# cvxgrp/qcqp

Measured on AMD Instinct MI355X. Metric: restarts x coord-sweeps / sec (improve COORD_DESCENT phase-2 sweeps, 2n^2 flops each; whole step timed), higher is better.
Workload: dtype f64

## Files before the change

qcqp_amd/csrc/cd_life.hip:

```cpp
#include "cd_life.h"

#include <cstdio>
#include <cstdlib>

#include "onevar.h"
#include "cd_phase1_sep.h"
#include "cd_chain.h"
#include "cd_roles.h"

namespace qcqpmi {
namespace {

constexpr int L2_WD = 1 << 21;
enum { L2_ABORT = 3 };

__device__ __attribute__((always_inline)) inline RqOwn l2_own(int NB, int CS, int m, int NMW) {
    RqOwn o;
    const int rest = NB - CS;
    o.NB = NB;
    if (m < 0) { o.first = rest; o.stride = 1; o.nu = CS; }
    else { o.first = m; o.stride = NMW; o.nu = m < rest ? (rest - m + NMW - 1) / NMW : 0; }
    return o;
}

constexpr int L2_SHARED_DOUBLES = 8 + 8 + 16 + 8;
constexpr int L2_YU = 6;
constexpr int l2_tile_doubles(int nmw, int csu, int lr, int kcl = 1, int maxc = 1) {
    return 2 * nmw * 256 + 256 + 256 + 2 * 256 + 2 * 48 + 4 * 256 + csu * 256 + 16 + 8 + 16 * 4 + 8 * 5 + 64 * 10 + 16 * 3 + 8 * 5 + 32 +
           (lr ? L2_YBMAX * 256 + 2 * 256 : 0) +
           2 * (maxc + 1) * 16 * kcl + 2 * 8 * kcl + (kcl > 1 ? 16 : 0);
}
#define L2_LDS_VIEW(tile_) \
    extern __shared__ double smem[]; \
    int *ctl = (int *)smem; \
    int *simdof = (int *)(smem + 8); \
    int *p1cols = (int *)(smem + 16); \
    int *jn = (int *)(smem + 32); \
    double *sp = smem + L2_SHARED_DOUBLES + (tile_) * l2_tile_doubles(NMW, CSU, LRV, KCLV, MAXC); \
    double *part2 = sp; sp += 2 * NMW * 256; \
    double *fixp = sp; sp += 256; \
    double *gtile = sp; sp += 256; \
    double *DU2 = sp; sp += 2 * 256; \
    double *sc2 = sp; sp += 2 * 48; \
    double *ring = sp; sp += 4 * 256; \
    double *cshare = sp; sp += CSU * 256; \
    double *slk = sp; sp += 16; \
    rq_lds_int *sy = (rq_lds_int *)(int *)sp; sp += 8; \
    double *of0 = sp; sp += 16; \
    long long *ovis = (long long *)sp; sp += 16; \
    long long *oacc = (long long *)sp; sp += 16; \
    long long *oswp = (long long *)sp; sp += 16; \
    int *sid = (int *)sp; sp += 8; \
    int *snew = (int *)sp; sp += 8; \
    int *sfin = (int *)sp; sp += 8; \
    int *ost = (int *)sp; sp += 8; \
    int *gatep = (int *)sp; sp += 8; \
    long long *cst = (long long *)sp; sp += 64 * 10; \
    unsigned long long *sseed = (unsigned long long *)sp; sp += 16; \
    unsigned long long *sfirst = (unsigned long long *)sp; sp += 16; \
    unsigned long long *p1key = (unsigned long long *)sp; sp += 16; \
    int *p1upd = (int *)sp; sp += 8; \
    int *p1fin = (int *)sp; sp += 8; \
    int *p1sw = (int *)sp; sp += 8; \
    int *p1st = (int *)sp; sp += 8; \
    L2Par *par = (L2Par *)sp; sp += 32;       \
    double *ytile = sp; sp += LRV ? L2_YBMAX * 256 : 0; \
    double *pend = sp; sp += LRV ? 2 * 256 : 0; \
    SetTable<MAXC> TC;        \
    TC.slots = 16 * KCLV; \
    TC.lo = sp; sp += (MAXC + 1) * 16 * KCLV; \
    TC.hi = sp; sp += (MAXC + 1) * 16 * KCLV; \
    TC.n = (int *)sp; sp += 8 * KCLV; \
    TC.slow = (int *)sp; sp += 8 * KCLV; \
    int *clsb = (int *)sp;
template <class T>
__device__ __attribute__((always_inline)) inline T *l2_tl(T *p, int t, int tile_doubles) { return (T *)((double *)p + t * tile_doubles); }

struct L2Par {
    const double *Apack, *Apack2, *Dpack, *Spack;
    const double *Gpack, *Upack;
    int RB, pad_;
    double *Xg;
    int *next;
    unsigned long long *prof;
    long long num_iters, n16;
    double tol, r0, fbound;
    int NB, KS, n, nlast, Rtotal, dbg;
    const int *cls;
};
static_assert(sizeof(L2Par) <= 32 * sizeof(double), "L2Par outgrew its LDS slot");
__device__ __attribute__((always_inline)) inline int l2_uni(int v) { return __builtin_amdgcn_readfirstlane(v); }
__device__ __attribute__((always_inline)) inline long long l2_uni(long long v) {
    const int lo = __builtin_amdgcn_readfirstlane((int)(v & 0xffffffffll)), hi = __builtin_amdgcn_readfirstlane((int)(v >> 32));
    return ((long long)hi << 32) | (long long)(unsigned)lo;
}
__device__ __attribute__((always_inline)) inline double l2_uni(double v) { return __longlong_as_double(l2_uni(__double_as_longlong(v))); }
template <class T>
__device__ __attribute__((always_inline)) inline T *l2_uni(T *p) { return (T *)(uintptr_t)l2_uni((long long)(uintptr_t)p); }

template <int NMW, int CS>
__device__ __attribute__((noinline)) void l2_mfma_role(int m_in, int t_in) {
    constexpr int MAXC = 1;
    constexpr int KCLV = 1;
    constexpr int CSU = CS > 0 ? CS : 1;
    constexpr int LRV = 0;
    const int tile = l2_uni(t_in);
    L2_LDS_VIEW(tile)
    (void)ytile; (void)pend; (void)clsb;
    (void)fixp; (void)gtile; (void)DU2; (void)sc2; (void)cshare; (void)slk; (void)TC; (void)of0; (void)ovis; (void)oacc; (void)oswp; (void)sid; (void)snew;
    (void)sfin; (void)ost; (void)ctl; (void)cst; (void)sseed; (void)sfirst; (void)p1key; (void)p1upd; (void)p1fin; (void)p1sw; (void)p1st; (void)gatep; (void)simdof; (void)p1cols; (void)jn;
    const int lane = threadIdx.x & 63;
    const int m = l2_uni(m_in);
    const double *pApack2 = l2_uni(par->Apack2);
    double *pXg = l2_uni(par->Xg);
    unsigned long long *pprof = l2_uni(par->prof);
    const int NB = l2_uni(par->NB), KS = l2_uni(par->KS);
    const int64_t n16 = l2_uni(par->n16);
    const int rowmask = (l2_uni(par->dbg) & 1) ? 7 : -1;
    const int64_t gmax = (int64_t)1 << 40;
    const RqOwn own = l2_own(NB, CS, m, NMW);
    const int nu = own.nu;
    v2d_ arP[2 * RQ_PFU];
    const unsigned vlane = (unsigned)lane * 16u;
    const __amdgpu_buffer_rsrc_t arsrc = __builtin_amdgcn_make_buffer_rsrc(const_cast<double *>(pApack2), 0, NB * KS * 512, 0x00020000);
    const __amdgpu_buffer_rsrc_t xrsrc = __builtin_amdgcn_make_buffer_rsrc(pXg, 0, (int)(n16 * 128), 0x00020000);
    const int rowstride = KS * 512;
    typedef unsigned rq_u4 __attribute__((ext_vector_type(4)));
    typedef unsigned rq_u2 __attribute__((ext_vector_type(2)));
    #define L2_LDA(dst, soff, vo) { const rq_u4 t0_ = __builtin_amdgcn_raw_buffer_load_b128(arsrc, (vo), (soff), 0);           \
                            const rq_u4 t1_ = __builtin_amdgcn_raw_buffer_load_b128(arsrc, (vo) + 1024u, (soff), 0);   \
                            (dst)[0] = __builtin_bit_cast(v2d_, t0_); (dst)[1] = __builtin_bit_cast(v2d_, t1_); }
    double bq[4 * RQ_PERS];
    {
        const unsigned vl8 = (unsigned)lane * 8u;
    #pragma unroll
        for (int u = 0; u < RQ_PERS; u++)
    #pragma unroll
            for (int q = 0; q < 4; q++) {
                const rq_u2 t_ = __builtin_amdgcn_raw_buffer_load_b64(xrsrc, vl8, (m + NMW * u) * 2048 + q * 512, 0);
                bq[4 * u + q] = __builtin_bit_cast(double, t_);
            }
    }
    typedef __attribute__((address_space(3))) const double rq_lds_cd;
    rq_lds_cd *rbase = (rq_lds_cd *)(ring + lane);
    asm volatile("" : "+v"(rbase));
    int row = 0;
    #pragma unroll
    for (int U = 0; U < RQ_PFU; U++) L2_LDA(arP + 2 * U, row * rowstride + (m + ((U < nu) ? NMW * U : 0)) * 2048, vlane)
    int spins = 0;
    const bool prof_on = pprof != nullptr && m == 0 && tile == 0;
    long long pw_commit = 0, pw_cons = 0;
    for (int64_t i = 0; i < gmax; i++) {
        const int row2 = (row + 1 == NB) ? 0 : row + 1;
        const int h1 = row == 0 ? NB - 1 : row - 1;
        const int h2 = h1 == 0 ? NB - 1 : h1 - 1;
        const int r1 = (i >= 3) ? (h2 == 0 ? NB - 1 : h2 - 1) : -1;
        unsigned skip = ~0u << own.nu, fresh = 0u;
        if (h1 % NMW == m && h1 < NB - CS) skip |= 1u << (h1 / NMW);
        if (h2 % NMW == m && h2 < NB - CS) skip |= 1u << (h2 / NMW);
        if (r1 >= 0 && r1 % NMW == m && r1 < NB - CS) fresh |= 1u << (r1 / NMW);
        const int so1 = (row & rowmask) * rowstride + m * 2048, so2 = (row2 & rowmask) * rowstride + m * 2048;
        bool stop = false;
        if (i >= 3) {
            const long long tw0 = prof_on ? (long long)__builtin_amdgcn_s_memtime() : 0;
            for (;;) {
                const rq_i4 s4 = rq_sync_read(sy);
                if (s4[RQ_STOP]) { stop = true; break; }
                if (s4[RQ_COMMIT] >= (int)i - 2) break;
                if (++spins > L2_WD) { stop = true; rq_sync_write(sy, L2_ABORT, 1, lane); rq_sync_write(sy, RQ_STOP, 1, lane); break; }
                __builtin_amdgcn_s_sleep(1);
            }
            if (stop) break;
            spins = 0;
            if (prof_on) pw_commit += (long long)__builtin_amdgcn_s_memtime() - tw0;
            if (fresh) {
                rq_lds_cd *rp = rbase + (int)((i - 3) & 3) * 256;
    #pragma unroll
                for (int u = 0; u < RQ_PERS; u++)
                    if ((fresh >> u) & 1u) {
    #pragma unroll
                        for (int q = 0; q < 4; q++) bq[4 * u + q] = rp[q * 64];
                    }
            }
        }
        v4d_ acc = {0.0, 0.0, 0.0, 0.0}, acc1 = acc;
    #pragma unroll
        for (int third = 0; third < RQ_RND; third++) {
    #pragma unroll
            for (int U = 0; U < RQ_PFU; U++) {
                const int u = RQ_PFU * third + U;
                if (u < RQ_MAXU && !((skip >> u) & 1u)) {
                    const double *bu = bq + 4 * u;
                    acc = __builtin_amdgcn_mfma_f64_16x16x4f64(arP[2 * U][0], bu[0], acc, 0, 0, 0);
                    acc1 = __builtin_amdgcn_mfma_f64_16x16x4f64(arP[2 * U][1], bu[1], acc1, 0, 0, 0);
                    acc = __builtin_amdgcn_mfma_f64_16x16x4f64(arP[2 * U + 1][0], bu[2], acc, 0, 0, 0);
                    acc1 = __builtin_amdgcn_mfma_f64_16x16x4f64(arP[2 * U + 1][1], bu[3], acc1, 0, 0, 0);
                }
                if (third < RQ_RND - 1) { if (u + RQ_PFU < RQ_MAXU) L2_LDA(arP + 2 * U, so1 + ((u + RQ_PFU < nu) ? NMW * 2048 * (u + RQ_PFU) : 0), vlane) }
                else L2_LDA(arP + 2 * U, so2 + ((U < nu) ? NMW * 2048 * U : 0), vlane)
            }
        }
        acc = acc + acc1;
        if (i >= 2) {
            const long long tw0 = prof_on ? (long long)__builtin_amdgcn_s_memtime() : 0;
            for (;;) {
                const rq_i4 s4 = rq_sync_read(sy);
                if (s4[RQ_STOP]) { stop = true; break; }
                if (s4[RQ_CONS] >= (int)i - 1) break;
                if (++spins > L2_WD) { stop = true; rq_sync_write(sy, L2_ABORT, 1, lane); rq_sync_write(sy, RQ_STOP, 1, lane); break; }
                __builtin_amdgcn_s_sleep(1);
            }
            if (stop) break;
            spins = 0;
            if (prof_on) pw_cons += (long long)__builtin_amdgcn_s_memtime() - tw0;
        }
        {
            double *part = part2 + (int)(i & 1) * NMW * 256 + m * 256;
    #pragma unroll
            for (int v = 0; v < 4; v++) part[v * 64 + (lane & 15) * 4 + (lane >> 4)] = acc[v];
        }
        rq_sync_write(sy, RQ_PARTS + m, (int)i + 1, lane);
        row = row2;
    }
    if (prof_on && lane == 0) {
        atomicAdd(pprof + 9, (unsigned long long)pw_commit);
        atomicAdd(pprof + 10, (unsigned long long)pw_cons);
    }
    #undef L2_LDA
}


template <int NMW>
__device__ __attribute__((noinline)) void l2_mfma_lr_role(int m_in, int t_in) {
    constexpr int MAXC = 1;
    constexpr int KCLV = 1;
    constexpr int CSU = 1;
    constexpr int LRV = 1;
    constexpr int YU = L2_YU;
    const int tile = l2_uni(t_in);
    L2_LDS_VIEW(tile)
    (void)clsb;
    (void)fixp; (void)gtile; (void)DU2; (void)sc2; (void)cshare; (void)slk; (void)TC; (void)of0; (void)ovis; (void)oacc; (void)oswp; (void)sid; (void)snew;
    (void)sfin; (void)ost; (void)ctl; (void)cst; (void)sseed; (void)sfirst; (void)p1key; (void)p1upd; (void)p1fin; (void)p1sw; (void)p1st; (void)gatep; (void)simdof; (void)p1cols; (void)jn;
// ... 560 lines not shown
                }
                double bqC[4 * CSU];
    #pragma unroll
                for (int U = 0; U < CSU; U++)
    #pragma unroll
                    for (int q = 0; q < 4; q++) bqC[4 * U + q] = cshare[U * 256 + q * 64 + lane];
                acc = rq_product<CSU>(arC, bqC, Apk2, KS, cown, lane, us, rq_slot(cown, bprev), bn2, acc);
            }
    #pragma unroll
            for (int v = 0; v < 4; v++) fixp[v * 64 + (lane & 15) * 4 + (lane >> 4)] = acc[v];
        }
        {
            const int nx = (int)((g + 1) & 1);
    #pragma unroll
            for (int e = 0; e < 4; e++) DU2[nx * 256 + lane + 64 * e] = d4[e];
            if (lane < 48) sc2[nx * 48 + lane] = s3;
            if (MULTI && lane < 16) clsb[nx * 16 + lane] = c3;
        }
        L2_TICK(pt_fix)
        b = bn;
    }
#undef L2_TICK
    if (LR) {
        const int g1 = (int)((last_g - 1) & 3), g0 = (int)(last_g & 3);
        double p1v[4], p0v[4];
#pragma unroll
        for (int u = 0; u < 4; u++) { p1v[u] = ring[g1 * 256 + u * 64 + lane]; p0v[u] = ring[g0 * 256 + u * 64 + lane]; }
#pragma unroll
        for (int u = 0; u < 4; u++) { pend[u * 64 + lane] = p1v[u]; pend[256 + u * 64 + lane] = p0v[u]; }
    }
    rq_sync_write(sy, RQ_STOP, 1, lane);
    if (prof_on && lane == 0) {
        atomicAdd(pprof + 13, (unsigned long long)pt_sum);
        atomicAdd(pprof + 14, (unsigned long long)pt_steps);
        atomicAdd(pprof + 15, (unsigned long long)pt_end);
        atomicAdd(pprof + 19, (unsigned long long)pt_req);
        *(long long *)(ctl + 8) = (long long)__builtin_amdgcn_s_memtime();
        atomicAdd(pprof + 7, (unsigned long long)pt_fix);
        atomicAdd(pprof + 8, (unsigned long long)pw_part);
        atomicAdd(pprof + 11, (unsigned long long)pn_int);
        atomicAdd(pprof + 12, (unsigned long long)pn_gen);
    }
    {
        cst[0 * 64 + lane] = S.upd_counter; cst[1 * 64 + lane] = S.visits; cst[2 * 64 + lane] = S.accepted;
        cst[3 * 64 + lane] = S.sweeps; cst[4 * 64 + lane] = S.conv ? 1 : 0; cst[5 * 64 + lane] = S.status;
        cst[6 * 64 + lane] = __double_as_longlong(fpart);
        cst[7 * 64 + lane] = (frz ? 1 : 0) | (done ? 2 : 0) | (pre ? 4 : 0) | (ld ? 8 : 0);
        cst[8 * 64 + lane] = __double_as_longlong(facc);
        const double ftot = rq_quad_sum(facc) + P.r0;
        const bool fin = occupied && done;
        if (gq == 0) {
            sfin[r] = fin ? 1 : 0;
            if (fin) { ovis[r] = S.visits; oacc[r] = S.accepted; oswp[r] = S.sweeps; ost[r] = S.status; of0[r] = ftot; }
        }
    }
    __builtin_amdgcn_s_setprio(0);
}

template <int NMW, int CS, int KIND, int TILES, int LR>
__global__ __launch_bounds__((NMW == 3 && TILES == 1) ? 256 : 512, 2) void cd_life_kernel(CdLife2Args a0) {
    const CdLife2Args &a = a0;
    constexpr bool MULTI = KIND == L2_KIND_GENK || KIND == L2_KIND_LINK;
    constexpr int BK = KIND == L2_KIND_GENK ? L2_KIND_GEN : KIND == L2_KIND_LINK ? L2_KIND_LIN : KIND;
    constexpr int MAXC = MULTI ? 2 : 1;
    constexpr int KCLV = MULTI ? L2_KCL : 1;
    constexpr int CSU = CS > 0 ? CS : 1;
    constexpr int LRV = LR;
    static_assert(!MULTI || (TILES == 1 && !LR), "multi-class kinds: one tile per workgroup, no objective factor");
    constexpr int NT = (NMW == 3 && TILES == 1) ? 256 : 512;
    constexpr int NW = NT / 64;
    constexpr int NS = 16 * TILES;
    constexpr int TD = l2_tile_doubles(NMW, CSU, LR);
    static_assert(!LR || (NMW == 3 && CS == 0 && BK != L2_KIND_LIN && BK != L2_KIND_SGN), "factored objective: three multiplying waves per tile, no chain share, a positive diagonal");
    constexpr bool PRE = BK == L2_KIND_LIN || BK == L2_KIND_SGN;
    static_assert(TILES == 1 || NMW == 3, "two tiles per workgroup: eight waves = two chains + two x three multiplying waves");
    const DevProblem &P = a.P;
    const int tid0 = threadIdx.x;
    const int wave = __builtin_amdgcn_readfirstlane(tid0 >> 6);
    const int64_t n16 = P.n16;
    const int NB = (int)P.NB, KS = (int)P.KS;
    L2_LDS_VIEW(0)
    (void)fixp; (void)gtile; (void)DU2; (void)sc2; (void)ring; (void)cshare; (void)of0; (void)ovis; (void)oacc; (void)oswp; (void)ost; (void)ytile; (void)pend; (void)clsb;
#define L2_STORE_SETS(st_, sc_, slack_) {                                                                                              \
        SetTable<MAXC> T2 = TC;                                                                                                          \
        T2.lo = l2_tl(TC.lo, st_, TD); T2.hi = l2_tl(TC.hi, st_, TD); T2.n = l2_tl(TC.n, st_, TD); T2.slow = l2_tl(TC.slow, st_, TD);    \
        const int nk_ = MULTI ? a0.nclass : 1;                                                                                           \
        for (int k_ = 0; k_ < nk_; k_++) {                                                                                               \
            FeasSet<MAXC> C_;                                                                                                            \
            compute_set<MAXC>(P, P.krep[k_], slack_, C_);                                                                                \
            store_set<MAXC>(T2, 16 * k_ + (sc_), C_);                                                                                    \
            if (MULTI && C_.n > 2) T2.slow[16 * k_ + (sc_)] = 1;                                                                         \
        }                                                                                                                                \
    }
    GLB double *Xg0 = glb(a0.scratch) + (int64_t)blockIdx.x * TILES * n16 * 16;

    if ((tid0 & 63) == 0) simdof[wave] = (int)(__builtin_amdgcn_s_getreg(4 | (4 << 6) | (1 << 11)));
    if (NMW == 3 && TILES == 1 && tid0 == 0) {
        int arrival = 0;
        if (a0.cuslot) {
            const unsigned hw = __builtin_amdgcn_s_getreg(4 | (0 << 6) | (31 << 11)), xcc = __builtin_amdgcn_s_getreg(20 | (0 << 6) | (31 << 11));
            arrival = glb_add(glb(a0.cuslot) + (((xcc & 15) << 8) | (((hw >> 12) & 15) << 4) | ((hw >> 8) & 15)), 1);
        }
        simdof[8] = (arrival & 1) ? (a0.rotmode == 2 ? 16 + 1 : 2) : 0;
    }
    if (tid0 < 64 * TILES) {
        long long *cs_ = l2_tl(cst, tid0 >> 6, TD);
#pragma unroll
        for (int f = 0; f < 10; f++) cs_[f * 64 + (tid0 & 63)] = (f == 4) ? 1 : 0;
    }
    if (tid0 < NS) { l2_tl(sid, tid0 >> 4, TD)[tid0 & 15] = -1; l2_tl(sfin, tid0 >> 4, TD)[tid0 & 15] = 0; }
    GLB const CdLife *lf0 = glb(a0.life);
    const long long life_t0 = (tid0 == 0 && lf0->prof) ? (long long)__builtin_amdgcn_s_memtime() : 0;
    __syncthreads();
    int role, rtile = 0;
    {
        int cnt[4] = {0, 0, 0, 0};
        int rank = 0;
        const int mys = simdof[wave];
#pragma unroll
        for (int w = 0; w < NW; w++) {
            const int s = simdof[w];
#pragma unroll
            for (int q = 0; q < 4; q++) cnt[q] += (s == q) ? 1 : 0;
            rank += (s == mys && w < wave) ? 1 : 0;
        }
        const bool even = cnt[0] == NW / 4 && cnt[1] == NW / 4 && cnt[2] == NW / 4 && cnt[3] == NW / 4;
        if (NMW == 3 && TILES == 1) {
            const int rot = simdof[8];
            if (!even) role = wave;
            else if (rot >= 16) role = mys == 0 ? 0 : 1 + ((mys - 1 + (rot - 16)) % 3);
            else role = (mys + rot) & 3;
        }
        else if (TILES == 2) { role = even ? mys : (wave & 3); rtile = even ? rank : (wave >> 2); }
        else if (even) role = (mys == 0) ? (rank == 0 ? 0 : 7) : mys + 3 * rank;
        else role = wave;
        role = __builtin_amdgcn_readfirstlane(role);
        rtile = __builtin_amdgcn_readfirstlane(rtile);
        if (tid0 == 0 && lf0->prof) {
            if (even) atomicAdd((unsigned long long *)lf0->prof + 6, 1ull);
            const unsigned hw = __builtin_amdgcn_s_getreg(4 | (0 << 6) | (31 << 11)), xcc = __builtin_amdgcn_s_getreg(20 | (0 << 6) | (31 << 11));
            Xg0[0] = (double)(((xcc & 15) << 8) | (((hw >> 13) & 7) << 4) | ((hw >> 8) & 15));
        }
    }
    const int nlast = (int)(P.n - 16 * (int64_t)(NB - 1));
    if (tid0 < TILES) {
        L2Par *pr = l2_tl(par, tid0, TD);
        pr->Apack = P.Apack; pr->Apack2 = P.Apack2; pr->Dpack = a0.Dpack; pr->Spack = a0.Spack;
        pr->Gpack = a0.Gpack; pr->Upack = a0.Upack; pr->RB = a0.RB; pr->pad_ = 0;
        pr->Xg = a0.scratch + ((int64_t)blockIdx.x * TILES + tid0) * n16 * 16; pr->next = a0.b.next; pr->prof = (unsigned long long *)lf0->prof;
        pr->num_iters = a.num_iters; pr->n16 = n16; pr->tol = a.tol; pr->r0 = P.r0; pr->fbound = a.fbound;
        pr->NB = NB; pr->KS = KS; pr->n = (int)P.n; pr->nlast = nlast; pr->Rtotal = (int)lf0->Rtotal; pr->dbg = a0.dbg;
        pr->cls = P.cls;
    }
    __syncthreads();

    for (;;) {
        int tid = tid0;
        asm volatile("" : "+v"(tid));
        const CdLife *lifep = a0.life;
        asm volatile("" : "+s"(lifep));
        const int lane = tid & 63, r = lane >> 2;
        if (tid == 0) { ctl[0] = 0; jn[0] = 0; jn[1] = 0; }
        __syncthreads();
        if (tid < NS) {
            const int st = tid >> 4, sc = tid & 15;
            int id = l2_tl(sid, st, TD)[sc], nw = 0;
            if (id < 0) {
                GLB const CdLife *lf = glb(lifep);
                const int idx = glb_add(glb(a0.b.next), 1);
                if (idx < (int)lf->Rtotal) {
                    id = idx; nw = 1;
                    const uint64_t pop = (uint64_t)idx / (uint64_t)lf->Rpop, rho = (uint64_t)idx % (uint64_t)lf->Rpop;
                    l2_tl(sseed, st, TD)[sc] = lf->seed + pop * lf->seed_stride;
                    l2_tl(sfirst, st, TD)[sc] = lf->first_index + pop * lf->first_stride + rho - (uint64_t)idx;
                }
            }
            l2_tl(sid, st, TD)[sc] = id; l2_tl(snew, st, TD)[sc] = nw;
            if (nw) { l2_tl(p1fin, st, TD)[sc] = 0; l2_tl(p1sw, st, TD)[sc] = 0; l2_tl(p1st, st, TD)[sc] = 0; l2_tl(gatep, st, TD)[sc] = 0; }
            if (id < 0) {
                l2_tl(slk, st, TD)[sc] = 0.0;
                L2_STORE_SETS(st, sc, 0.0)
            }
            if (id >= 0) atomicAdd(&ctl[0], 1);
            *(volatile rq_lds_int *)(l2_tl((int *)sy, st, TD) + sc) = (sc >= RQ_PARTS + NMW) ? 0x7fffffff : 0;
        }
        __syncthreads();
        if (ctl[0] == 0) break;
        {
            __builtin_amdgcn_s_setprio(3);
            GLB const CdLife *lf = glb(lifep);
            const long long pt0 = lf->prof ? (long long)__builtin_amdgcn_s_memtime() : 0;
            const int lf_pre = LR ? lf->prebuilt : 0;
            const int lf_generate = lf->generate && !lf_pre, lf_phase1 = lf->phase1 && !lf_pre;
            const double lf_viol_tol = lf->viol_tol;
            const int e0 = P.cptr[P.krep[0]];
            const double cp = P.cp[e0], cq = P.cq[e0], cr = P.cr[e0];
            const int rel = P.crel[e0];
            for (int c = 0; c < NS; c++) {
                const int ct = c >> 4, cc = c & 15;
                GLB double *Xg = Xg0 + (int64_t)ct * n16 * 16;
                if (!l2_tl(snew, ct, TD)[cc]) {
                    if (l2_tl(sid, ct, TD)[cc] < 0) for (int64_t j = tid; j < n16; j += NT) Xg[j * 16 + cc] = 0.0;
                    continue;
                }
                if (!lf_generate) {
                    const int id = l2_tl(sid, ct, TD)[cc];
                    GLB const double *src = glb(a0.b.X) + ((int64_t)(id >> 4) * n16) * 16 + (id & 15);
                    for (int64_t j0 = tid; j0 < n16; j0 += 4 * NT) {
                        double t4[4];
#pragma unroll
                        for (int u = 0; u < 4; u++) t4[u] = (j0 + u * NT < n16) ? src[(j0 + u * NT) * 16] : 0.0;
#pragma unroll
                        for (int u = 0; u < 4; u++) if (j0 + u * NT < n16) Xg[(j0 + u * NT) * 16 + cc] = t4[u];
                    }
                }
            }
            if (lf_generate) {
                if (tid == 0) {
                    int cnt = 0;
                    for (int k = 0; k < NS; k++) if (l2_tl(snew, k >> 4, TD)[k & 15]) p1cols[cnt++] = k;
                    ctl[4] = cnt; ctl[5] = 0;
                }
                __syncthreads();
                const int ncolg = ctl[4], nchg = (int)((n16 + 127) / 128);
                for (;;) {
                    int ch = 0;
                    if (lane == 0) ch = atomicAdd(&ctl[5], 1);
                    ch = __builtin_amdgcn_readfirstlane(ch);
                    if (ch >= ncolg * nchg) break;
                    const int c = p1cols[ch / nchg], ct = c >> 4, cc = c & 15;
                    GLB double *Xg = Xg0 + (int64_t)ct * n16 * 16;
                    const int64_t j = (int64_t)(ch % nchg) * 128 + 2 * lane;
                    const uint64_t sd = l2_tl(sseed, ct, TD)[cc], gidx = l2_tl(sfirst, ct, TD)[cc] + (uint64_t)l2_tl(sid, ct, TD)[cc];
                    if (j < n16) {
                        double xo = 0.0;
                        const double xe = (j < P.n) ? keyed_normal_pair(sd, gidx, (uint64_t)j, &xo) : 0.0;
                        Xg[j * 16 + cc] = xe;
                        Xg[(j + 1) * 16 + cc] = (j + 1 < P.n) ? xo : 0.0;
                    }
                }
            }
            __syncthreads();
            if (lf->prof && tid == 0) atomicAdd((unsigned long long *)lf->prof + 4, (unsigned long long)((long long)__builtin_amdgcn_s_memtime() - pt0));
            if (lf_phase1) {
                const bool band2 = !MULTI && cq == 0.0 && rel == RELOP_EQ && cp > 1e-4 && cr < -1e-3;
                const int cw = band2 ? 128 : 64;
                const int nch = (int)((P.n + cw - 1) / cw);
                for (int64_t t = 0; t < a.num_iters; t++) {
                    if (tid == 0) {
                        int cnt = 0;
                        for (int k = 0; k < NS; k++) if (l2_tl(snew, k >> 4, TD)[k & 15] && !l2_tl(p1fin, k >> 4, TD)[k & 15]) p1cols[cnt++] = k;
                        ctl[4] = cnt; ctl[5] = 0;
                    }
                    if (tid < NS) { l2_tl(p1key, tid >> 4, TD)[tid & 15] = ordered_key(-QM_INF); l2_tl(p1upd, tid >> 4, TD)[tid & 15] = 0; }
                    __syncthreads();
                    const int ncol1 = ctl[4];
                    if (ncol1 == 0) break;
                    for (;;) {
                        int ch = 0;
                        if (lane == 0) ch = atomicAdd(&ctl[5], 1);
                        ch = __builtin_amdgcn_readfirstlane(ch);
                        if (ch >= ncol1 * nch) break;
                        const int c = p1cols[ch / nch], ct = c >> 4, cc = c & 15;
                        GLB double *Xg = Xg0 + (int64_t)ct * n16 * 16;
                        const uint64_t sd = l2_tl(sseed, ct, TD)[cc], gidx = l2_tl(sfirst, ct, TD)[cc] + (uint64_t)l2_tl(sid, ct, TD)[cc];
                        double va = -QM_INF;
                        int fl = 0;
                        if (band2) {
                            const int64_t i2[2] = {(int64_t)(ch % nch) * 128 + lane, (int64_t)(ch % nch) * 128 + 64 + lane};
                            const bool on2[2] = {i2[0] < P.n, i2[1] < P.n};
                            double x2[2] = {on2[0] ? Xg[i2[0] * 16 + cc] : 1.0, on2[1] ? Xg[i2[1] * 16 + cc] : 1.0};
                            P1Visit V2[2];
                            p1_band_visit_n<2>(cp, cq, cr, i2, x2, on2, a.tol, lf_viol_tol, sd, gidx, t, V2);
#pragma unroll
                            for (int k = 0; k < 2; k++)
                                if (on2[k]) {
                                    if (V2[k].moved) { Xg[i2[k] * 16 + cc] = x2[k]; fl |= 1; }
                                    if (V2[k].status) fl |= (-V2[k].status) << 8;
                                    va = V2[k].vafter > va ? V2[k].vafter : va;
                                }
                        } else {
                            const int64_t i = (int64_t)(ch % nch) * 64 + lane;
                            if (i < P.n) {
                                if (MULTI) {
                                    double xi = Xg[i * 16 + cc];
                                    P1Visit V;
                                    p1_sep_visit<MAXC>(P, i, xi, a.tol, lf_viol_tol, sd, gidx, t, V);
                                    fl = (V.moved ? 1 : 0) | ((-V.status) << 8);
                                    va = V.vafter;
                                    if (V.moved) Xg[i * 16 + cc] = xi;
                                } else {
                                    const double xi = p1_class_visit(cp, cq, cr, rel, i, Xg[i * 16 + cc], a.tol, lf_viol_tol, sd, gidx, t, &fl, &va);
                                    if (fl & 1) Xg[i * 16 + cc] = xi;
                                }
                            }
                        }
                        const double vmax = wave_max(va);
                        const bool anyupd = __builtin_amdgcn_ballot_w64((fl & 1) != 0) != 0ull;
                        const int st = (fl >> 8) ? -(fl >> 8) : 0;
                        if (lane == 0) { atomicMax(&l2_tl(p1key, ct, TD)[cc], ordered_key(vmax)); if (anyupd) l2_tl(p1upd, ct, TD)[cc] = 1; }
                        if (st) l2_tl(p1st, ct, TD)[cc] = st;
                    }
                    __syncthreads();
                    if (tid < NS && l2_tl(snew, tid >> 4, TD)[tid & 15] && !l2_tl(p1fin, tid >> 4, TD)[tid & 15]) {
                        const int st = tid >> 4, sc = tid & 15;
                        l2_tl(p1sw, st, TD)[sc]++;
                        if (ordered_unkey(l2_tl(p1key, st, TD)[sc]) < lf_viol_tol || !l2_tl(p1upd, st, TD)[sc]) l2_tl(p1fin, st, TD)[sc] = 1;
                    }
                    __syncthreads();
                }
            }
            if (lf->prof && tid == 0) atomicAdd((unsigned long long *)lf->prof + 17, (unsigned long long)((long long)__builtin_amdgcn_s_memtime() - pt0));
            if (tid < NS) l2_tl(p1key, tid >> 4, TD)[tid & 15] = ordered_key(-QM_INF);
            __syncthreads();
            for (int c = 0; c < NS; c++) {
                const int ct = c >> 4, cc = c & 15;
                if (lf_pre || !l2_tl(snew, ct, TD)[cc]) continue;
                GLB const double *Xg = Xg0 + (int64_t)ct * n16 * 16;
                double v = -QM_INF;
                for (int64_t i = tid; i < P.n; i += NT) {
                    const double x = Xg[i * 16 + cc];
                    if (MULTI) {
                        for (int e = P.cptr[i]; e < P.cptr[i + 1]; e++) {
                            const double f = (P.cp[e] * x + P.cq[e]) * x + P.cr[e];
                            const double w = viol_of(f, P.crel[e]);
                            v = w > v ? w : v;
                        }
                    } else {
                        const double f = (cp * x + cq) * x + cr;
                        const double w = (rel == RELOP_EQ) ? fabs(f) : (f > 0.0 ? f : 0.0);
                        v = w > v ? w : v;
                    }
                }
                v = wave_max(v);
                if (lane == 0) atomicMax(&l2_tl(p1key, ct, TD)[cc], ordered_key(v));
            }
            __syncthreads();
            if (tid < NS && l2_tl(snew, tid >> 4, TD)[tid & 15]) {
                const int st = tid >> 4, sc = tid & 15;
                double mvx;
                if (lf_pre) {
                    const int id = l2_tl(sid, st, TD)[sc];
                    mvx = glb(lf->preslack)[id];
                    l2_tl(p1sw, st, TD)[sc] = (int)glb(lf->sweeps1)[id];
                    l2_tl(p1st, st, TD)[sc] = glb(lf->status1)[id];
                    l2_tl(gatep, st, TD)[sc] = glb(lf->ran2)[id];
                } else {
                    mvx = ordered_unkey(l2_tl(p1key, st, TD)[sc]);
                    l2_tl(gatep, st, TD)[sc] = (mvx < lf_viol_tol && l2_tl(p1st, st, TD)[sc] == 0) ? 1 : 0;
                }
                l2_tl(slk, st, TD)[sc] = mvx;
                L2_STORE_SETS(st, sc, mvx)
            }
            __syncthreads();
            if (nlast < 16) {
                for (int w = tid; w < NS * (16 - nlast); w += NT) {
                    const int c = w % NS, ct = c >> 4, cc = c & 15, row = w / NS;
                    if (l2_tl(snew, ct, TD)[cc] || l2_tl(sid, ct, TD)[cc] < 0) {
                        const int nn = l2_tl(TC.n, ct, TD)[cc];
                        double xp = 0.0;
                        if (BK == L2_KIND_BAND) xp = nn >= 2 ? l2_tl(TC.lo, ct, TD)[16 * KCLV + cc] : 0.0;
                        else if (BK == L2_KIND_GEN) xp = nn >= 1 ? l2_tl(TC.hi, ct, TD)[cc] : 0.0;
                        else xp = nn >= 2 ? l2_tl(TC.hi, ct, TD)[16 * KCLV + cc] : l2_tl(TC.hi, ct, TD)[cc];
                        if (!(xp == xp) || __builtin_isinf(xp)) xp = 0.0;
                        (Xg0 + (int64_t)ct * n16 * 16)[(P.n + row) * 16 + cc] = xp;
                    }
                }
                __syncthreads();
            }
            if (LR) {
                const int r16 = 16 * a0.RB;
                const int y0n = lf_pre ? (int)lf->y0_count : 0;
                GLB const double *y0g = glb(lf->y0);
                for (int w = tid; w < NS * (32 + r16); w += NT) {
                    const int c = w % NS, ct = c >> 4, cc = c & 15, rowz = w / NS;
                    const int id = l2_tl(sid, ct, TD)[cc];
                    if (l2_tl(snew, ct, TD)[cc] || id < 0) {
                        double v = 0.0;
                        if (id >= 0 && id < y0n)
                            v = rowz < 32 ? (Xg0 + (int64_t)ct * n16 * 16)[(16 * (int64_t)(NB - 2) + rowz) * 16 + cc]
                                          : y0g[((int64_t)(id >> 4) * r16 + (rowz - 32)) * 16 + (id & 15)];
                        if (rowz < 32) l2_tl(pend, ct, TD)[rowz * 16 + cc] = v;
                        else l2_tl(ytile, ct, TD)[(rowz - 32) * 16 + cc] = v;
                    }
                }
                __syncthreads();
            }
            if (lf->prof && tid == 0) {
                int nn = 0;
                for (int k = 0; k < NS; k++) nn += l2_tl(snew, k >> 4, TD)[k & 15] ? 1 : 0;
                atomicAdd((unsigned long long *)lf->prof + 0, (unsigned long long)((long long)__builtin_amdgcn_s_memtime() - pt0));
                atomicAdd((unsigned long long *)lf->prof + 2, 1ull);
                atomicAdd((unsigned long long *)lf->prof + 3, (unsigned long long)nn);
            }
            __builtin_amdgcn_s_setprio(0);
        }
        if (role == 0) {
            long long *cs_ = l2_tl(cst, rtile, TD);
            if (l2_tl(snew, rtile, TD)[r]) {
#pragma unroll
                for (int f = 0; f < 6; f++) cs_[f * 64 + lane] = 0;
                const int pass = l2_tl(gatep, rtile, TD)[r];
                bool load = LR != 0;
                if (LR) {
                    GLB const CdLife *lf = glb(lifep);
                    if (lf->prebuilt && l2_tl(sid, rtile, TD)[r] < (int)lf->y0_count) load = false;
                }
                cs_[6 * 64 + lane] = 0;
                cs_[4 * 64 + lane] = (pass && !PRE && !load) ? 0 : 1;
                cs_[7 * 64 + lane] = (pass ? (PRE ? 4 : 0) : 1) | (load ? 8 : 0);
                cs_[8 * 64 + lane] = 0;
            } else if (l2_tl(sid, rtile, TD)[r] < 0) {
                cs_[4 * 64 + lane] = 1; cs_[6 * 64 + lane] = 0;
                cs_[7 * 64 + lane] = 2; cs_[8 * 64 + lane] = 0;
            }
        }
        __syncthreads();
        if (tid == 0 && glb(lifep)->prof) *(long long *)(ctl + 6) = (long long)__builtin_amdgcn_s_memtime();

        if (role > 0) {
            if (LR) l2_mfma_lr_role<NMW>(role - 1, rtile);
            else l2_mfma_role<NMW, CS>(role - 1, rtile);
        } else l2_chain_role<NMW, CS, KIND, TILES, LR>(rtile);

        __syncthreads();
        if (sy[L2_ABORT] || (TILES > 1 && l2_tl((int *)sy, 1, TD)[L2_ABORT])) {
            if (tid == 0) __hip_atomic_store(glb(a0.abort), 1, __ATOMIC_RELAXED, __HIP_MEMORY_SCOPE_AGENT);
            break;
        }
        if (tid == 0 && glb(lifep)->prof)
        {
            const long long now_ = (long long)__builtin_amdgcn_s_memtime();
            atomicAdd((unsigned long long *)glb(lifep)->prof + 5, (unsigned long long)(now_ - *(long long *)(ctl + 6)));
            atomicAdd((unsigned long long *)glb(lifep)->prof + 20, (unsigned long long)(now_ - *(long long *)(ctl + 8)));
        }
        {
            const int e0 = P.cptr[P.krep[0]];
            const double cp = P.cp[e0], cq = P.cq[e0], cr = P.cr[e0];
            const int rel = P.crel[e0];
            if (tid == 0) { int cnt = 0; for (int k = 0; k < NS; k++) if (l2_tl(sfin, k >> 4, TD)[k & 15]) p1cols[cnt++] = k; ctl[4] = cnt; }
            if (tid < NS) l2_tl(p1key, tid >> 4, TD)[tid & 15] = ordered_key(-QM_INF);
            __syncthreads();
            const int nfin = ctl[4];
            const int64_t items = (int64_t)nfin * n16;
            for (int64_t w0 = tid; w0 < items; w0 += (int64_t)NT * 8) {
                double xv8[8];
#pragma unroll
                for (int u = 0; u < 8; u++) {
                    const int64_t w = w0 + (int64_t)NT * u;
                    const int col = p1cols[w < items ? w / n16 : 0];
                    const int64_t i = w % n16;
                    xv8[u] = (w < items && i < P.n) ? (Xg0 + (int64_t)(col >> 4) * n16 * 16)[i * 16 + (col & 15)] : 0.0;
                }
#pragma unroll
                for (int u = 0; u < 8; u++) {
                    const int64_t w = w0 + (int64_t)NT * u;
                    if (w < items) {
                        const int col = p1cols[w / n16], id = l2_tl(sid, col >> 4, TD)[col & 15];
                        const int64_t i = w % n16;
                        glb(a0.b.X)[((int64_t)(id >> 4) * n16 + i) * 16 + (id & 15)] = xv8[u];
                        if (i < P.n) {
                            if (MULTI) {
                                double vv = -QM_INF;
                                for (int e = P.cptr[i]; e < P.cptr[i + 1]; e++) {
                                    const double w_ = viol_of((P.cp[e] * xv8[u] + P.cq[e]) * xv8[u] + P.cr[e], P.crel[e]);
                                    vv = w_ > vv ? w_ : vv;
                                }
                                atomicMax(&l2_tl(p1key, col >> 4, TD)[col & 15], ordered_key(vv));
                            } else {
                                const double f = (cp * xv8[u] + cq) * xv8[u] + cr;
                                const double vv = (rel == RELOP_EQ) ? fabs(f) : (f > 0.0 ? f : 0.0);
                                atomicMax(&l2_tl(p1key, col >> 4, TD)[col & 15], ordered_key(vv));
                            }
                        }
                    }
                }
            }
            __syncthreads();
            if (tid < NS && l2_tl(sfin, tid >> 4, TD)[tid & 15]) {
                const int st = tid >> 4, sc = tid & 15;
                const double mx = ordered_unkey(l2_tl(p1key, st, TD)[sc]);
                const int id = l2_tl(sid, st, TD)[sc];
                glb(a0.b.visits)[id] = l2_tl(ovis, st, TD)[sc]; glb(a0.b.accepted)[id] = l2_tl(oacc, st, TD)[sc]; glb(a0.b.sweeps)[id] = l2_tl(oswp, st, TD)[sc];
                glb(a0.b.status)[id] = l2_tl(ost, st, TD)[sc];
                if (a0.b.f0out) glb(a0.b.f0out)[id] = l2_tl(of0, st, TD)[sc];
                if (a0.b.mvout) glb(a0.b.mvout)[id] = mx;
                GLB const CdLife *lf = glb(lifep);
                glb(lf->sweeps1)[id] = l2_tl(p1sw, st, TD)[sc]; glb(lf->status1)[id] = l2_tl(p1st, st, TD)[sc];
                glb(lf->ran2)[id] = (uint8_t)l2_tl(gatep, st, TD)[sc];
                l2_tl(sid, st, TD)[sc] = -1; l2_tl(sfin, st, TD)[sc] = 0;
            }
            __syncthreads();
        }
    }
    if (tid0 == 0 && lf0->prof) {
        const unsigned long long dtl = (unsigned long long)((long long)__builtin_amdgcn_s_memtime() - life_t0);
        atomicAdd((unsigned long long *)lf0->prof + 1, dtl);
        atomicMax((unsigned long long *)lf0->prof + 16, dtl);
    }
}

#undef L2_STORE_SETS

constexpr int L2P_NT = 256;
__global__ __launch_bounds__(L2P_NT, 3) void cd_life_prep_kernel(DevProblem P, const CdLife *life, double *X, int64_t num_iters, double tol) {
    __shared__ unsigned long long key[16], csd[16], cgi[16];
    __shared__ int upd[16], st1[16], fin[16], sw[16], cols[16], nact;
    const int tid = threadIdx.x, s = tid & 15, g = tid >> 4;
    GLB const CdLife *lf = glb(life);
    const int64_t id = (int64_t)blockIdx.x * 16 + s;
    const bool valid = id < lf->Rtotal;
    const int64_t n = P.n, n16 = P.n16;
    GLB double *Xt = glb(X) + (int64_t)blockIdx.x * n16 * 16 + s;
    const double viol_tol = lf->viol_tol;
    uint64_t sd = 0, gidx = 0;
    if (valid) {
        const uint64_t pop = (uint64_t)id / (uint64_t)lf->Rpop, rho = (uint64_t)id % (uint64_t)lf->Rpop;
        sd = lf->seed + pop * lf->seed_stride;
        gidx = lf->first_index + pop * lf->first_stride + rho;
    }
    if (lf->generate && valid) {
        for (int64_t j = 2 * g; j < n16; j += 32) {
            double xo = 0.0;
            const double xe = (j < n) ? keyed_normal_pair(sd, gidx, (uint64_t)j, &xo) : 0.0;
            Xt[16 * j] = xe;
            Xt[16 * (j + 1)] = (j + 1 < n) ? xo : 0.0;
        }
    }
    const int e0 = P.cptr[P.krep[0]];
    const double cp = P.cp[e0], cq = P.cq[e0], cr = P.cr[e0];
    const int rel = P.crel[e0];
    if (tid < 16) { fin[tid] = valid ? 0 : 1; sw[tid] = 0; st1[tid] = 0; csd[tid] = sd; cgi[tid] = gidx; }
    if (lf->phase1) {
        const bool band2 = cq == 0.0 && rel == RELOP_EQ && cp > 1e-4 && cr < -1e-3;
        GLB double *Xtile = glb(X) + (int64_t)blockIdx.x * n16 * 16;
        for (int64_t t = 0; t < num_iters; t++) {
            if (tid < 16) { key[tid] = ordered_key(-QM_INF); upd[tid] = 0; }
            __syncthreads();
            if (tid == 0) { int c = 0; for (int k = 0; k < 16; k++) if (!fin[k]) cols[c++] = k; nact = c; }
            __syncthreads();
            if (nact == 0) break;
            const bool compact = t > 0 && nact < 16;
            const int npass = compact ? nact : 1;
            const int64_t j0 = compact ? 2 * tid : 2 * g, jstep = compact ? 2 * L2P_NT : 32;
            for (int qq = 0; qq < npass; qq++) {
                const int c = compact ? cols[qq] : s;
                const bool live = compact || !fin[s];
                GLB double *Xc = Xtile + c;
                const uint64_t sdc = csd[c], gic = cgi[c];
                double va = -QM_INF;
                int moved = 0, stv = 0;
                if (live) {
                    for (int64_t j = j0; j < n; j += jstep) {
                        if (band2) {
                            const int64_t i2[2] = {j, j + 1};
                            const bool on2[2] = {true, j + 1 < n};
                            double x2[2] = {Xc[16 * j], on2[1] ? Xc[16 * (j + 1)] : 1.0};
                            P1Visit V2[2];
                            p1_band_visit_n<2, true>(cp, cq, cr, i2, x2, on2, tol, viol_tol, sdc, gic, t, V2);
#pragma unroll
                            for (int k = 0; k < 2; k++)
                                if (on2[k]) {
                                    if (V2[k].moved) { Xc[16 * i2[k]] = x2[k]; moved = 1; }
                                    if (V2[k].status) stv = V2[k].status;
                                    va = V2[k].vafter > va ? V2[k].vafter : va;
                                }
                        } else {
                            for (int64_t i = j; i < j + 2 && i < n; i++) {
                                int fl = 0;
                                double v = 0.0;
                                const double xi = p1_class_visit(cp, cq, cr, rel, i, Xc[16 * i], tol, viol_tol, sdc, gic, t, &fl, &v);
                                if (fl & 1) { Xc[16 * i] = xi; moved = 1; }
                                if (fl >> 8) stv = -(fl >> 8);
                                va = v > va ? v : va;
                            }
                        }
                    }
                }
#pragma unroll
                for (int o = 16; o <= 32; o <<= 1) {
                    const double w = __shfl_xor(va, o, 64);
                    va = w > va ? w : va;
                    moved |= __shfl_xor(moved, o, 64);
                }
                if (compact) {
#pragma unroll
                    for (int o = 1; o <= 8; o <<= 1) {
                        const double w = __shfl_xor(va, o, 64);
                        va = w > va ? w : va;
// ... 208 lines not shown
```

Measured before the change: 29.22 million.

## Fuse restart turnover into one pass with LDS-cached life params

```diff
diff --git a/qcqp_amd/csrc/cd_life.hip b/qcqp_amd/csrc/cd_life.hip
--- a/qcqp_amd/csrc/cd_life.hip
+++ b/qcqp_amd/csrc/cd_life.hip
@@ -89,6 +89,19 @@
     const int *cls;
 };
 static_assert(sizeof(L2Par) <= 32 * sizeof(double), "L2Par outgrew its LDS slot");
+struct L2Life {
+    int64_t Rtotal, Rpop, y0_count;
+    uint64_t seed, seed_stride, first_index, first_stride;
+    const double *preslack, *y0;
+    int64_t *sweeps1;
+    int *status1;
+    uint8_t *ran2;
+    unsigned long long *prof;
+    double cp, cq, cr;
+    int rel, prebuilt;
+    int turn, pad_;
+};
+static_assert(sizeof(L2Life) <= 256, "L2Life outgrew the tail of the LDS allocation");
 __device__ __attribute__((always_inline)) inline int l2_uni(int v) { return __builtin_amdgcn_readfirstlane(v); }
 __device__ __attribute__((always_inline)) inline long long l2_uni(long long v) {
     const int lo = __builtin_amdgcn_readfirstlane((int)(v & 0xffffffffll)), hi = __builtin_amdgcn_readfirstlane((int)(v >> 32));
@@ -955,6 +968,19 @@
         pr->NB = NB; pr->KS = KS; pr->n = (int)P.n; pr->nlast = nlast; pr->Rtotal = (int)lf0->Rtotal; pr->dbg = a0.dbg;
         pr->cls = P.cls;
     }
+    L2Life *const lfl = (L2Life *)(smem + L2_SHARED_DOUBLES + TILES * TD);
+    (void)lfl;
+    if constexpr (LR != 0) {
+        if (tid0 == 0) {
+            lfl->Rtotal = lf0->Rtotal; lfl->Rpop = lf0->Rpop; lfl->y0_count = lf0->y0_count;
+            lfl->seed = lf0->seed; lfl->seed_stride = lf0->seed_stride; lfl->first_index = lf0->first_index; lfl->first_stride = lf0->first_stride;
+            lfl->preslack = lf0->preslack; lfl->y0 = lf0->y0; lfl->sweeps1 = lf0->sweeps1; lfl->status1 = lf0->status1; lfl->ran2 = lf0->ran2;
+            lfl->prof = (unsigned long long *)lf0->prof; lfl->prebuilt = lf0->prebuilt;
+            const int e0 = P.cptr[P.krep[0]];
+            lfl->cp = P.cp[e0]; lfl->cq = P.cq[e0]; lfl->cr = P.cr[e0]; lfl->rel = P.crel[e0];
+            lfl->turn = (lf0->prebuilt && lf0->Rtotal > (int64_t)gridDim.x * NS) ? 1 : 0; lfl->pad_ = 0;
+        }
+    }
     __syncthreads();
 
     for (;;) {
@@ -963,33 +989,179 @@
         const CdLife *lifep = a0.life;
         asm volatile("" : "+s"(lifep));
         const int lane = tid & 63, r = lane >> 2;
-        if (tid == 0) { ctl[0] = 0; jn[0] = 0; jn[1] = 0; }
-        __syncthreads();
-        if (tid < NS) {
-            const int st = tid >> 4, sc = tid & 15;
-            int id = l2_tl(sid, st, TD)[sc], nw = 0;
-            if (id < 0) {
-                GLB const CdLife *lf = glb(lifep);
-                const int idx = glb_add(glb(a0.b.next), 1);
-                if (idx < (int)lf->Rtotal) {
-                    id = idx; nw = 1;
-                    const uint64_t pop = (uint64_t)idx / (uint64_t)lf->Rpop, rho = (uint64_t)idx % (uint64_t)lf->Rpop;
-                    l2_tl(sseed, st, TD)[sc] = lf->seed + pop * lf->seed_stride;
-                    l2_tl(sfirst, st, TD)[sc] = lf->first_index + pop * lf->first_stride + rho - (uint64_t)idx;
-                }
-            }
-            l2_tl(sid, st, TD)[sc] = id; l2_tl(snew, st, TD)[sc] = nw;
-            if (nw) { l2_tl(p1fin, st, TD)[sc] = 0; l2_tl(p1sw, st, TD)[sc] = 0; l2_tl(p1st, st, TD)[sc] = 0; l2_tl(gatep, st, TD)[sc] = 0; }
-            if (id < 0) {
-                l2_tl(slk, st, TD)[sc] = 0.0;
-                L2_STORE_SETS(st, sc, 0.0)
-            }
-            if (id >= 0) atomicAdd(&ctl[0], 1);
-            *(volatile rq_lds_int *)(l2_tl((int *)sy, st, TD) + sc) = (sc >= RQ_PARTS + NMW) ? 0x7fffffff : 0;
-        }
-        __syncthreads();
-        if (ctl[0] == 0) break;
-        {
+        bool turned = false;
+        if constexpr (LR != 0) {
+            if (l2_uni(lfl->turn)) {
+                turned = true;
+                __builtin_amdgcn_s_setprio(3);
+                unsigned long long *const profp = l2_uni(lfl->prof);
+                const long long pt0 = profp ? (long long)__builtin_amdgcn_s_memtime() : 0;
+                const int r16 = 16 * a0.RB;
+                const int y0n = (int)l2_uni((long long)lfl->y0_count);
+                int oldid = -1, idv = -1, nwv = 0, nnew = 0;
+                double nslack = 0.0;
+                long long nsw1 = 0;
+                int nst1 = 0, nran2 = 0;
+                if (tid < NS) {
+                    const int st = tid >> 4, sc = tid & 15;
+                    int id = l2_tl(sid, st, TD)[sc];
+                    if (l2_tl(sfin, st, TD)[sc]) {
+                        oldid = id; id = -1;
+                        glb(a0.b.visits)[oldid] = l2_tl(ovis, st, TD)[sc]; glb(a0.b.accepted)[oldid] = l2_tl(oacc, st, TD)[sc]; glb(a0.b.sweeps)[oldid] = l2_tl(oswp, st, TD)[sc];
+                        glb(a0.b.status)[oldid] = l2_tl(ost, st, TD)[sc];
+                        if (a0.b.f0out) glb(a0.b.f0out)[oldid] = l2_tl(of0, st, TD)[sc];
+                        glb(lfl->sweeps1)[oldid] = l2_tl(p1sw, st, TD)[sc]; glb(lfl->status1)[oldid] = l2_tl(p1st, st, TD)[sc];
+                        glb(lfl->ran2)[oldid] = (uint8_t)l2_tl(gatep, st, TD)[sc];
+                        l2_tl(sfin, st, TD)[sc] = 0;
+                    }
+                    if (id < 0) {
+                        const int idx = glb_add(glb(a0.b.next), 1);
+                        if (idx < (int)lfl->Rtotal) {
+                            id = idx; nwv = 1;
+                            nslack = glb(lfl->preslack)[idx]; nsw1 = glb(lfl->sweeps1)[idx]; nst1 = glb(lfl->status1)[idx]; nran2 = glb(lfl->ran2)[idx];
+                            const uint64_t pop = (uint64_t)idx / (uint64_t)lfl->Rpop, rho = (uint64_t)idx % (uint64_t)lfl->Rpop;
+                            l2_tl(sseed, st, TD)[sc] = lfl->seed + pop * lfl->seed_stride;
+                            l2_tl(sfirst, st, TD)[sc] = lfl->first_index + pop * lfl->first_stride + rho - (uint64_t)idx;
+                        }
+                    }
+                    idv = id;
+                    l2_tl(sid, st, TD)[sc] = id; l2_tl(snew, st, TD)[sc] = nwv; l2_tl(p1upd, st, TD)[sc] = oldid;
+                    l2_tl(p1key, st, TD)[sc] = ordered_key(-QM_INF);
+                    *(volatile rq_lds_int *)(l2_tl((int *)sy, st, TD) + sc) = (sc >= RQ_PARTS + NMW) ? 0x7fffffff : 0;
+                    const unsigned long long mturn = __builtin_amdgcn_ballot_w64(oldid >= 0 || nwv || id < 0);
+                    const unsigned long long mocc = __builtin_amdgcn_ballot_w64(id >= 0), mnew = __builtin_amdgcn_ballot_w64(nwv != 0);
+                    if (oldid >= 0 || nwv || id < 0) p1cols[__builtin_popcountll(mturn & ((1ull << tid) - 1ull))] = tid;
+                    nnew = __builtin_popcountll(mnew);
+                    if (tid == 0) { ctl[0] = __builtin_popcountll(mocc); ctl[4] = __builtin_popcountll(mturn); jn[0] = 0; jn[1] = 0; }
+                }
+                __syncthreads();
+                {
+                    const double cp = l2_uni(lfl->cp), cq = l2_uni(lfl->cq), cr = l2_uni(lfl->cr);
+                    const int rel = l2_uni(lfl->rel);
+                    GLB const double *y0g = glb(l2_uni(lfl->y0));
+                    const int nturn = l2_uni(ctl[4]);
+                    const int KR = (int)((n16 + NT - 1) / NT), KI = KR + (r16 + NT - 1) / NT;
+                    const int np = (int)P.n, nx = (int)n16;
+                    constexpr int L2_TCH = 16;
+                    double vacc = -QM_INF;
+                    int ci0 = 0, k0 = 0;
+                    while (ci0 < nturn) {
+                        double xo[L2_TCH], xn[L2_TCH];
+                        int ci = ci0, k = k0;
+#pragma unroll
+                        for (int q = 0; q < L2_TCH; q++) {
+                            xo[q] = 0.0; xn[q] = 0.0;
+                            if (ci < nturn) {
+                                const int c = l2_uni(p1cols[ci]), ct = c >> 4, cc = c & 15;
+                                const int oid = l2_uni(l2_tl(p1upd, ct, TD)[cc]), id = l2_uni(l2_tl(sid, ct, TD)[cc]), nw = l2_uni(l2_tl(snew, ct, TD)[cc]);
+                                if (k < KR) {
+                                    const int j = k * NT + tid;
+                                    if (oid >= 0 && j < np) xo[q] = (Xg0 + (int64_t)ct * n16 * 16)[(int64_t)j * 16 + cc];
+                                    if (nw && j < nx) xn[q] = glb(a0.b.X)[((int64_t)(id >> 4) * n16 + j) * 16 + (id & 15)];
+                                } else {
+                                    const int row = (k - KR) * NT + tid;
+                                    if (nw && id < y0n && row < r16) xn[q] = y0g[((int64_t)(id >> 4) * r16 + row) * 16 + (id & 15)];
+                                }
+                                if (++k == KI) { k = 0; ci++; }
+                            }
+                        }
+                        ci = ci0; k = k0;
+#pragma unroll
+                        for (int q = 0; q < L2_TCH; q++) {
+                            if (ci < nturn) {
+                                const int c = l2_uni(p1cols[ci]), ct = c >> 4, cc = c & 15;
+                                const int oid = l2_uni(l2_tl(p1upd, ct, TD)[cc]), id = l2_uni(l2_tl(sid, ct, TD)[cc]), nw = l2_uni(l2_tl(snew, ct, TD)[cc]);
+                                if (k < KR) {
+                                    const int j = k * NT + tid;
+                                    if (oid >= 0) {
+                                        if (j < nx) glb(a0.b.X)[((int64_t)(oid >> 4) * n16 + j) * 16 + (oid & 15)] = xo[q];
+                                        if (j < np) {
+                                            const double f = (cp * xo[q] + cq) * xo[q] + cr;
+                                            const double vv = (rel == RELOP_EQ) ? fabs(f) : (f > 0.0 ? f : 0.0);
+                                            vacc = vv > vacc ? vv : vacc;
+                                        }
+                                        if (k == KR - 1) {
+                                            const double vw = wave_max(vacc);
+                                            if (lane == 0) atomicMax(&l2_tl(p1key, ct, TD)[cc], ordered_key(vw));
+                                            vacc = -QM_INF;
+                                        }
+                                    }
+                                    if ((nw || id < 0) && j < nx) {
+                                        (Xg0 + (int64_t)ct * n16 * 16)[(int64_t)j * 16 + cc] = xn[q];
+                                        if (j >= nx - 32) l2_tl(pend, ct, TD)[(j - (nx - 32)) * 16 + cc] = (nw && id < y0n) ? xn[q] : 0.0;
+                                    }
+                                } else {
+                                    const int row = (k - KR) * NT + tid;
+                                    if ((nw || id < 0) && row < r16) l2_tl(ytile, ct, TD)[row * 16 + cc] = xn[q];
+                                }
+                                if (++k == KI) { k = 0; ci++; }
+                            }
+                        }
+                        ci0 = ci; k0 = k;
+                    }
+                }
+                if (tid < NS && (nwv || idv < 0)) {
+                    const int st = tid >> 4, sc = tid & 15;
+                    if (nwv) { l2_tl(p1fin, st, TD)[sc] = 0; l2_tl(p1sw, st, TD)[sc] = (int)nsw1; l2_tl(p1st, st, TD)[sc] = nst1; l2_tl(gatep, st, TD)[sc] = nran2; }
+                    l2_tl(slk, st, TD)[sc] = nslack;
+                    L2_STORE_SETS(st, sc, nslack)
+                }
+                __syncthreads();
+                if (tid < NS && oldid >= 0 && a0.b.mvout) glb(a0.b.mvout)[oldid] = ordered_unkey(l2_tl(p1key, tid >> 4, TD)[tid & 15]);
+                if (ctl[0] == 0) break;
+                if (nlast < 16) {
+                    for (int w = tid; w < NS * (16 - nlast); w += NT) {
+                        const int c = w % NS, ct = c >> 4, cc = c & 15, row = w / NS;
+                        const int id = l2_tl(sid, ct, TD)[cc];
+                        if (l2_tl(snew, ct, TD)[cc] || id < 0) {
+                            const int nn = l2_tl(TC.n, ct, TD)[cc];
+                            double xp = 0.0;
+                            static_assert(BK == L2_KIND_BAND || BK == L2_KIND_GEN, "turnover pass: padding fixed point of the band and gen kinds only");
+                            if (BK == L2_KIND_BAND) xp = nn >= 2 ? l2_tl(TC.lo, ct, TD)[16 * KCLV + cc] : 0.0;
+                            else xp = nn >= 1 ? l2_tl(TC.hi, ct, TD)[cc] : 0.0;
+                            if (!(xp == xp) || __builtin_isinf(xp)) xp = 0.0;
+                            (Xg0 + (int64_t)ct * n16 * 16)[(P.n + row) * 16 + cc] = xp;
+                            l2_tl(pend, ct, TD)[(16 + nlast + row) * 16 + cc] = (id >= 0 && id < y0n) ? xp : 0.0;
+                        }
+                    }
+                }
+                if (profp && tid == 0) {
+                    atomicAdd(profp + 0, (unsigned long long)((long long)__builtin_amdgcn_s_memtime() - pt0));
+                    atomicAdd(profp + 2, 1ull);
+                    atomicAdd(profp + 3, (unsigned long long)nnew);
+                }
+                __builtin_amdgcn_s_setprio(0);
+            }
+        }
+        if (!turned) {
+            if (tid == 0) { ctl[0] = 0; jn[0] = 0; jn[1] = 0; }
+            __syncthreads();
+            if (tid < NS) {
+                const int st = tid >> 4, sc = tid & 15;
+                int id = l2_tl(sid, st, TD)[sc], nw = 0;
+                if (id < 0) {
+                    GLB const CdLife *lf = glb(lifep);
+                    const int idx = glb_add(glb(a0.b.next), 1);
+                    if (idx < (int)lf->Rtotal) {
+                        id = idx; nw = 1;
+                        const uint64_t pop = (uint64_t)idx / (uint64_t)lf->Rpop, rho = (uint64_t)idx % (uint64_t)lf->Rpop;
+                        l2_tl(sseed, st, TD)[sc] = lf->seed + pop * lf->seed_stride;
+                        l2_tl(sfirst, st, TD)[sc] = lf->first_index + pop * lf->first_stride + rho - (uint64_t)idx;
+                    }
+                }
+                l2_tl(sid, st, TD)[sc] = id; l2_tl(snew, st, TD)[sc] = nw;
+                if (nw) { l2_tl(p1fin, st, TD)[sc] = 0; l2_tl(p1sw, st, TD)[sc] = 0; l2_tl(p1st, st, TD)[sc] = 0; l2_tl(gatep, st, TD)[sc] = 0; }
+                if (id < 0) {
+                    l2_tl(slk, st, TD)[sc] = 0.0;
+                    L2_STORE_SETS(st, sc, 0.0)
+                }
+                if (id >= 0) atomicAdd(&ctl[0], 1);
+                *(volatile rq_lds_int *)(l2_tl((int *)sy, st, TD) + sc) = (sc >= RQ_PARTS + NMW) ? 0x7fffffff : 0;
+            }
+            __syncthreads();
+            if (ctl[0] == 0) break;
+        }
+        if (!turned) {
             __builtin_amdgcn_s_setprio(3);
             GLB const CdLife *lf = glb(lifep);
             const long long pt0 = lf->prof ? (long long)__builtin_amdgcn_s_memtime() : 0;
@@ -1205,9 +1377,8 @@
                 for (int f = 0; f < 6; f++) cs_[f * 64 + lane] = 0;
                 const int pass = l2_tl(gatep, rtile, TD)[r];
                 bool load = LR != 0;
-                if (LR) {
-                    GLB const CdLife *lf = glb(lifep);
-                    if (lf->prebuilt && l2_tl(sid, rtile, TD)[r] < (int)lf->y0_count) load = false;
+                if constexpr (LR != 0) {
+                    if (lfl->prebuilt && l2_tl(sid, rtile, TD)[r] < (int)lfl->y0_count) load = false;
                 }
                 cs_[6 * 64 + lane] = 0;
                 cs_[4 * 64 + lane] = (pass && !PRE && !load) ? 0 : 1;
@@ -1219,7 +1390,9 @@
             }
         }
         __syncthreads();
-        if (tid == 0 && glb(lifep)->prof) *(long long *)(ctl + 6) = (long long)__builtin_amdgcn_s_memtime();
+        if constexpr (LR != 0) {
+            if (tid == 0 && lfl->prof) *(long long *)(ctl + 6) = (long long)__builtin_amdgcn_s_memtime();
+        } else if (tid == 0 && glb(lifep)->prof) *(long long *)(ctl + 6) = (long long)__builtin_amdgcn_s_memtime();
 
         if (role > 0) {
             if (LR) l2_mfma_lr_role<NMW>(role - 1, rtile);
@@ -1231,13 +1404,19 @@
             if (tid == 0) __hip_atomic_store(glb(a0.abort), 1, __ATOMIC_RELAXED, __HIP_MEMORY_SCOPE_AGENT);
             break;
         }
-        if (tid == 0 && glb(lifep)->prof)
+        if constexpr (LR != 0) {
+            if (tid == 0 && lfl->prof) {
+                const long long now_ = (long long)__builtin_amdgcn_s_memtime();
+                atomicAdd(lfl->prof + 5, (unsigned long long)(now_ - *(long long *)(ctl + 6)));
+                atomicAdd(lfl->prof + 20, (unsigned long long)(now_ - *(long long *)(ctl + 8)));
+            }
+        } else if (tid == 0 && glb(lifep)->prof)
         {
             const long long now_ = (long long)__builtin_amdgcn_s_memtime();
             atomicAdd((unsigned long long *)glb(lifep)->prof + 5, (unsigned long long)(now_ - *(long long *)(ctl + 6)));
             atomicAdd((unsigned long long *)glb(lifep)->prof + 20, (unsigned long long)(now_ - *(long long *)(ctl + 8)));
         }
-        {
+        if (!turned) {
             const int e0 = P.cptr[P.krep[0]];
             const double cp = P.cp[e0], cq = P.cq[e0], cr = P.cr[e0];
             const int rel = P.crel[e0];
```

After: 30.24 million (median of 6 runs). +3.5%, better.
